# wjqkkky/TTS

Hardware: AMD Instinct MI355X
Metric: mel-frames/s (Tacotron2-DDC + MB-MelGAN end-to-end) (higher is better)
Workload: dtype f32; 1 GPU; C2: Tacotron2-DDC (r_init=7, r=2, sigmoid attn) + MB-MelGAN [8,4,2]x4, 32 LJ-length utterances per GPU; global_batch=32, r=2, parallelism=replicas x1

## Files before the change

### include/ttship.h

```cpp
#ifndef TTSHIP_H
#define TTSHIP_H

#include <stdint.h>

#ifdef __cplusplus
extern "C" {
#endif

typedef struct tts_ctx tts_ctx;

int tts_version(void);
const char* tts_last_error(void);

int tts_ctx_create(int device, tts_ctx** out);
int tts_ctx_destroy(tts_ctx* ctx);

int tts_taco_set_tensor(tts_ctx* ctx, const char* name, const float* h_data, const int64_t* shape, int ndim);
int tts_taco_finalize(tts_ctx* ctx, int num_chars, int r_init, int attn_norm);

int tts_taco_infer(tts_ctx* ctx, const int64_t* d_ids, const int32_t* h_lens, int B, int T_max, int r,
                   const int32_t* h_max_steps, int S_cap, float stop_threshold, float* d_dec, float* d_post,
                   float* d_align, float* d_stop, int32_t* h_steps, int32_t* h_status, void* stream);

int tts_taco_infer_spk(tts_ctx* ctx, const int64_t* d_ids, const int32_t* h_lens, int B, int T_max, int r,
// ... 85 lines not shown
                      int use_lstm_with_projection);
int tts_ge2e_infer(tts_ctx* ctx, const float* d_x, const int32_t* h_lens, int B, int T_max, float* d_out,
                   void* stream);

int tts_mel_to_linear(tts_ctx* ctx, const float* d_mel, const int32_t* h_lens, int B, int M_max, int n_mels,
                      int n_freq, const float* d_inv_basis, const float* d_scale, const float* d_offset,
                      float clip_lo, float clip_hi, int use_clip, float spec_gain, float power, float* d_S,
                      void* stream);

int tts_griffin_lim(tts_ctx* ctx, const float* d_S, const int32_t* h_lens, int B, int M_max, int n_fft,
                    int win_length, int hop_length, int iters, const float* d_phase0, float* d_wav, void* stream);

int tts_stft_mag(tts_ctx* ctx, const float* d_wav, const int32_t* h_nsamples, int B, int L_max, int n_fft,
                 int win_length, int hop_length, float preemphasis, int algo, float* d_mag, int M_max,
                 void* stream);

int tts_mag_to_feature(tts_ctx* ctx, const float* d_mag, const int32_t* h_lens, int B, int M_max, int n_freq,
                       int n_out, const float* d_basis, float spec_gain, const float* d_scale,
                       const float* d_offset, float clip_lo, float clip_hi, int use_clip, float* d_out,
                       void* stream);

int tts_spec_to_mag(tts_ctx* ctx, const float* d_spec, const int32_t* h_lens, int B, int M_max, int n_freq,
                    const float* d_scale, const float* d_offset, float clip_lo, float clip_hi, int use_clip,
                    float spec_gain, float power, float* d_S, void* stream);

int tts_deemphasis(tts_ctx* ctx, const float* d_in, const int32_t* h_nsamples, int B, int L_max, double a,
                   float* d_out, void* stream);

int tts_wav_finish(tts_ctx* ctx, const float* d_wav, const int32_t* h_nsamples, int B, int L_max,
                   int window_length, int hop_length, double threshold, int gap, int16_t* d_pcm, int32_t* d_ends,
                   int32_t* d_total, void* stream);

int tts_time_decoder_kernel(tts_ctx* ctx, int which, int iters, float* ms_out);

int tts_decoder_stats(tts_ctx* ctx, int* path, int* nlaunch, float* ms, int* steps);

int tts_set_gemm_mode(tts_ctx* ctx, int mode);
int tts_gemm_mode(tts_ctx* ctx, int* mode, int64_t* fallbacks);

int tts_taco_mbmelgan_infer(tts_ctx* ctx, const int64_t* d_ids, const int32_t* h_lens, int B, int T_max, int r,
                            const int32_t* h_max_steps, int S_cap, float thr, const int64_t* d_spk_ids,
                            const float* d_spk_emb, float* d_dec, float* d_post, float* d_align, float* d_stop,
                            int pad, float* d_wav, int32_t* h_steps, int32_t* h_status, void* stream);

int tts_taco_mbmelgan_submit(tts_ctx* ctx, const int64_t* d_ids, const int32_t* h_lens, int B, int T_max, int r,
                             const int32_t* h_max_steps, int S_cap, float thr, const int64_t* d_spk_ids,
                             const float* d_spk_emb, float* d_dec, float* d_post, float* d_align, float* d_stop,
                             int pad, float* d_wav, int32_t* h_steps, int32_t* h_status, int64_t* h_ticket,
                             void* stream);
int tts_taco_mbmelgan_finish(tts_ctx* ctx, int64_t ticket, void* stream);

int tts_test_stall_lstm(int recurrence);

#ifdef __cplusplus
}
#endif
#endif
```

### tts_amd/_lib.py

```python

import atexit
import collections
import ctypes
import os
import threading
from typing import Dict

import numpy as np

_HERE = os.path.dirname(os.path.abspath(__file__))
LIB_PATH = os.environ.get("TTSHIP_LIB", os.path.join(_HERE, "libttship.so"))

_lib = None
_lock = threading.Lock()

_c_int_p = ctypes.POINTER(ctypes.c_int32)
_c_i64_p = ctypes.POINTER(ctypes.c_int64)
_c_f_p = ctypes.POINTER(ctypes.c_float)
_c_i_p = ctypes.POINTER(ctypes.c_int)
_vp = ctypes.c_void_p

SIGNATURES = [
    ("tts_version", ctypes.c_int, []),
    ("tts_last_error", ctypes.c_char_p, []),
# ... 16 lines not shown
                                            _c_int_p, _vp]),
    ("tts_taco_forward_style", ctypes.c_int, [_vp, _vp, _c_int_p, ctypes.c_int, ctypes.c_int, ctypes.c_int, _vp,
                                              _c_int_p, ctypes.c_int, _vp, _vp, _vp, _vp, _vp, _vp, _vp, _vp]),
    ("tts_taco_mbmelgan_infer", ctypes.c_int, [_vp, _vp, _c_int_p, ctypes.c_int, ctypes.c_int, ctypes.c_int,
                                               _c_int_p, ctypes.c_int, ctypes.c_float, _vp, _vp, _vp, _vp, _vp,
                                               _vp, ctypes.c_int, _vp, _c_int_p, _c_int_p, _vp]),
    ("tts_taco_mbmelgan_submit", ctypes.c_int, [_vp, _vp, _c_int_p, ctypes.c_int, ctypes.c_int, ctypes.c_int,
                                                _c_int_p, ctypes.c_int, ctypes.c_float, _vp, _vp, _vp, _vp, _vp,
                                                _vp, ctypes.c_int, _vp, _c_int_p, _c_int_p, _c_i64_p, _vp]),
    ("tts_taco_mbmelgan_finish", ctypes.c_int, [_vp, ctypes.c_int64, _vp]),
    ("tts_taco_speaker_dim", ctypes.c_int, [_vp, _c_i_p, _c_i_p]),
    ("tts_taco_set_options", ctypes.c_int, [_vp, ctypes.c_int, ctypes.c_int, ctypes.c_int]),
    ("tts_taco_encoder", ctypes.c_int, [_vp, _vp, _c_int_p, ctypes.c_int, ctypes.c_int, _vp, _vp]),
    ("tts_taco_postnet", ctypes.c_int, [_vp, _vp, _c_int_p, ctypes.c_int, ctypes.c_int, _vp, _vp]),
    ("tts_taco_decoder_state", ctypes.c_int, [_vp, ctypes.c_int, ctypes.c_int, _vp, _vp, _vp, _vp, _vp, _vp, _vp, _vp]),
    ("tts_tacotron1_set_tensor", ctypes.c_int, [_vp, ctypes.c_char_p, _vp, _c_i64_p, ctypes.c_int]),
    ("tts_tacotron1_finalize", ctypes.c_int, [_vp, ctypes.c_int, ctypes.c_int, ctypes.c_int, ctypes.c_int,
                                              ctypes.c_int]),
    ("tts_tacotron1_infer", ctypes.c_int, [_vp, _vp, _c_int_p, ctypes.c_int, ctypes.c_int, ctypes.c_int, _c_int_p,
                                           ctypes.c_int, _vp, _vp, _vp, _vp, _c_int_p, _c_int_p, _vp]),
    ("tts_tacotron1_encoder", ctypes.c_int, [_vp, _vp, _c_int_p, ctypes.c_int, ctypes.c_int, _vp, _vp]),
    ("tts_tacotron1_postnet", ctypes.c_int, [_vp, _vp, _c_int_p, ctypes.c_int, ctypes.c_int, _vp, _vp]),
    ("tts_melgan_set_tensor", ctypes.c_int, [_vp, ctypes.c_char_p, _vp, _c_i64_p, ctypes.c_int]),
    ("tts_melgan_finalize", ctypes.c_int, [_vp, ctypes.c_int, ctypes.c_int, ctypes.c_int, _c_int_p, ctypes.c_int,
                                           ctypes.c_int, ctypes.c_int]),
    ("tts_melgan_infer", ctypes.c_int, [_vp, _vp, _c_int_p, ctypes.c_int, ctypes.c_int, ctypes.c_int, _vp, _vp]),
    ("tts_melgan_infer_strided", ctypes.c_int, [_vp, _vp, ctypes.c_int64, ctypes.c_int64, ctypes.c_int64, _c_int_p,
                                                ctypes.c_int, ctypes.c_int, ctypes.c_int, _vp, _vp]),
    ("tts_melgan_generator", ctypes.c_int, [_vp, _vp, _c_int_p, ctypes.c_int, ctypes.c_int, ctypes.c_int, _vp,
                                            _vp]),
    ("tts_pqmf_synthesis", ctypes.c_int, [_vp, _vp, ctypes.c_int, ctypes.c_int, ctypes.c_int, _vp, ctypes.c_int,
                                          _vp, _vp]),
    ("tts_ge2e_set_tensor", ctypes.c_int, [_vp, ctypes.c_char_p, _vp, _c_i64_p, ctypes.c_int]),
    ("tts_ge2e_finalize", ctypes.c_int, [_vp, ctypes.c_int, ctypes.c_int, ctypes.c_int, ctypes.c_int,
                                         ctypes.c_int]),
    ("tts_ge2e_infer", ctypes.c_int, [_vp, _vp, _c_int_p, ctypes.c_int, ctypes.c_int, _vp, _vp]),
    ("tts_pwgan_set_tensor", ctypes.c_int, [_vp, ctypes.c_char_p, _vp, _c_i64_p, ctypes.c_int]),
    ("tts_pwgan_finalize", ctypes.c_int, [_vp, ctypes.c_int, ctypes.c_int, _c_int_p, ctypes.c_int]),
    ("tts_pwgan_infer", ctypes.c_int, [_vp, _vp, _c_int_p, ctypes.c_int, ctypes.c_int, ctypes.c_int, _vp, _vp,
                                       _vp]),
    ("tts_glow_set_tensor", ctypes.c_int, [_vp, ctypes.c_char_p, _vp, _c_i64_p, ctypes.c_int]),
    ("tts_glow_finalize", ctypes.c_int, [_vp, ctypes.c_int, ctypes.c_int, ctypes.c_int, ctypes.c_int]),
    ("tts_glow_encode", ctypes.c_int, [_vp, _vp, _c_int_p, ctypes.c_int, ctypes.c_int, ctypes.c_float, _c_int_p,
                                       _vp]),
    ("tts_glow_encode_spk", ctypes.c_int, [_vp, _vp, _c_int_p, _c_int_p, ctypes.c_int, ctypes.c_int, ctypes.c_float,
                                           _c_int_p, _vp]),
    ("tts_glow_decode", ctypes.c_int, [_vp, _vp, ctypes.c_float, ctypes.c_int, _vp, _vp, _vp, _vp, _vp]),
    ("tts_glow_align", ctypes.c_int, [_vp, _vp, _c_int_p, ctypes.c_int, _vp, _vp, _vp, _vp, _vp, _vp, _vp, _vp]),
    ("tts_glow_mas", ctypes.c_int, [_vp, _vp, _c_int_p, _c_int_p, ctypes.c_int, ctypes.c_int, ctypes.c_int, _vp, _vp]),
    ("tts_time_decoder_kernel", ctypes.c_int, [_vp, ctypes.c_int, ctypes.c_int, _c_f_p]),
    ("tts_decoder_stats", ctypes.c_int, [_vp, _c_i_p, _c_i_p, _c_f_p, _c_i_p]),
    ("tts_set_gemm_mode", ctypes.c_int, [_vp, ctypes.c_int]),
    ("tts_test_stall_lstm", ctypes.c_int, [ctypes.c_int]),
    ("tts_gemm_mode", ctypes.c_int, [_vp, _c_i_p, _c_i64_p]),
    ("tts_mel_to_linear", ctypes.c_int, [_vp, _vp, _c_int_p, ctypes.c_int, ctypes.c_int, ctypes.c_int, ctypes.c_int,
                                         _vp, _vp, _vp, ctypes.c_float, ctypes.c_float, ctypes.c_int, ctypes.c_float,
                                         ctypes.c_float, _vp, _vp]),
    ("tts_griffin_lim", ctypes.c_int, [_vp, _vp, _c_int_p, ctypes.c_int, ctypes.c_int, ctypes.c_int, ctypes.c_int,
                                       ctypes.c_int, ctypes.c_int, _vp, _vp, _vp]),
    ("tts_stft_mag", ctypes.c_int, [_vp, _vp, _c_int_p, ctypes.c_int, ctypes.c_int, ctypes.c_int, ctypes.c_int,
                                    ctypes.c_int, ctypes.c_float, ctypes.c_int, _vp, ctypes.c_int, _vp]),
    ("tts_mag_to_feature", ctypes.c_int, [_vp, _vp, _c_int_p, ctypes.c_int, ctypes.c_int, ctypes.c_int, ctypes.c_int,
                                          _vp, ctypes.c_float, _vp, _vp, ctypes.c_float, ctypes.c_float, ctypes.c_int,
                                          _vp, _vp]),
    ("tts_spec_to_mag", ctypes.c_int, [_vp, _vp, _c_int_p, ctypes.c_int, ctypes.c_int, ctypes.c_int, _vp, _vp,
                                       ctypes.c_float, ctypes.c_float, ctypes.c_int, ctypes.c_float, ctypes.c_float,
                                       _vp, _vp]),
    ("tts_deemphasis", ctypes.c_int, [_vp, _vp, _c_int_p, ctypes.c_int, ctypes.c_int, ctypes.c_double, _vp, _vp]),
    ("tts_wav_finish", ctypes.c_int, [_vp, _vp, _c_int_p, ctypes.c_int, ctypes.c_int, ctypes.c_int, ctypes.c_int,
                                      ctypes.c_double, ctypes.c_int, _vp, _vp, _vp, _vp]),
]


def load_library():
    global _lib
    with _lock:
        if _lib is None:
            if not os.path.exists(LIB_PATH):
                raise RuntimeError(f"libttship.so not found at {LIB_PATH}; run __graft_entry__.build() "
                                   f"(make -C tts_amd/csrc)")
            lib = ctypes.CDLL(LIB_PATH)
            for name, res, args in SIGNATURES:
                fn = getattr(lib, name)
                fn.restype = res
                fn.argtypes = args
            _lib = lib
    return _lib


def _check(rc: int):
    if rc != 0:
        msg = load_library().tts_last_error()
        raise RuntimeError("ttship: " + (msg.decode() if msg else "unknown error"))


def _i32(a):
    arr = np.ascontiguousarray(np.asarray(a, dtype=np.int32))
    return arr, arr.ctypes.data_as(_c_int_p)


def _ptr(t):
    return ctypes.c_void_p(t.data_ptr())


def _opt_ptr(t):
    return None if t is None else _ptr(t)
# ... 246 lines not shown
        B, N, L = x.shape
        taps = G.shape[-1] - 1
        _check(self.lib.tts_pqmf_synthesis(self.h, _ptr(x), B, N, L, _ptr(G), taps, _ptr(y), _stream(x.device)))

    def mel_to_linear(self, mel, lens, inv_basis, scale, offset, clip, spec_gain, power, S):
        B, M, n_mels = mel.shape
        lens_a, lens_p = _i32(lens)
        lo, hi = (0.0, 0.0) if clip is None else clip
        _check(self.lib.tts_mel_to_linear(self.h, _ptr(mel), lens_p, B, M, n_mels, S.shape[-1], _ptr(inv_basis),
                                          _ptr(scale), _ptr(offset), float(lo), float(hi), int(clip is not None),
                                          float(spec_gain), float(power), _ptr(S), _stream(mel.device)))

    def griffin_lim(self, S, lens, n_fft, win_length, hop_length, iters, phase0, wav):
        B, M, _ = S.shape
        lens_a, lens_p = _i32(lens)
        _check(self.lib.tts_griffin_lim(self.h, _ptr(S), lens_p, B, M, int(n_fft), int(win_length), int(hop_length),
                                        int(iters), _ptr(phase0), _ptr(wav), _stream(S.device)))

    def stft_mag(self, wav, nsamples, n_fft, win_length, hop_length, preemphasis, mag, algo=0):
        B, L = wav.shape
        n_a, n_p = _i32(nsamples)
        _check(self.lib.tts_stft_mag(self.h, _ptr(wav), n_p, B, L, int(n_fft), int(win_length), int(hop_length),
                                     float(preemphasis), int(algo), _ptr(mag), mag.shape[1], _stream(wav.device)))

    def mag_to_feature(self, mag, lens, basis, spec_gain, scale, offset, clip, out):
        B, M, n_freq = mag.shape
        lens_a, lens_p = _i32(lens)
        lo, hi = (0.0, 0.0) if clip is None else clip
        _check(self.lib.tts_mag_to_feature(self.h, _ptr(mag), lens_p, B, M, n_freq, out.shape[-1],
                                           None if basis is None else _ptr(basis), float(spec_gain), _ptr(scale),
                                           _ptr(offset), float(lo), float(hi), int(clip is not None), _ptr(out),
                                           _stream(mag.device)))

    def spec_to_mag(self, spec, lens, scale, offset, clip, spec_gain, power, S):
        B, M, n_freq = spec.shape
        lens_a, lens_p = _i32(lens)
        lo, hi = (0.0, 0.0) if clip is None else clip
        _check(self.lib.tts_spec_to_mag(self.h, _ptr(spec), lens_p, B, M, n_freq, _ptr(scale), _ptr(offset),
                                        float(lo), float(hi), int(clip is not None), float(spec_gain), float(power),
                                        _ptr(S), _stream(spec.device)))

    def deemphasis(self, wav, nsamples, a, out):
        B, L = wav.shape
        n_a, n_p = _i32(nsamples)
        _check(self.lib.tts_deemphasis(self.h, _ptr(wav), n_p, B, L, float(a), _ptr(out), _stream(wav.device)))

    def wav_finish(self, wav, nsamples, window_length, hop_length, threshold, gap, pcm, ends, total):
        B, L = wav.shape
        n_a, n_p = _i32(nsamples)
        _check(self.lib.tts_wav_finish(self.h, _ptr(wav), n_p, B, L, int(window_length), int(hop_length),
                                       float(threshold), int(gap), _ptr(pcm), _ptr(ends), _ptr(total),
                                       _stream(wav.device)))

    def decoder_stats(self):
        path, n = ctypes.c_int(0), ctypes.c_int(0)
        ms = (ctypes.c_float * 4)()
        st = (ctypes.c_int * 4)()
        _check(self.lib.tts_decoder_stats(self.h, ctypes.byref(path), ctypes.byref(n), ms, st))
        return int(path.value), [(float(ms[i]), int(st[i])) for i in range(n.value)]

    def set_gemm_mode(self, mode: str):
        if mode not in ("x3", "f32"):
            raise ValueError("gemm mode must be 'x3' or 'f32'")
        with self.lock:
            _check(self.lib.tts_set_gemm_mode(self.h, 1 if mode == "x3" else 0))

    def gemm_mode(self):
        m, n = ctypes.c_int(0), ctypes.c_int64(0)
        _check(self.lib.tts_gemm_mode(self.h, ctypes.byref(m), ctypes.byref(n)))
        return ("x3" if m.value else "f32"), int(n.value)

    def time_decoder_kernel(self, which: int, iters: int) -> float:
        ms = ctypes.c_float(0.0)
        _check(self.lib.tts_time_decoder_kernel(self.h, which, iters, ctypes.byref(ms)))
        return float(ms.value)


_engines: Dict[int, Engine] = {}


def get_engine(device) -> Engine:
    import torch
    dev = torch.device(device)
    if dev.type != "cuda":
        raise RuntimeError("tts_amd runs on MI355X (ROCm 'cuda' devices) only; got device "
                           f"'{dev}'. There is no CPU fallback: move the model with .cuda().")
    idx = dev.index if dev.index is not None else torch.cuda.current_device()
    with _lock:
        eng = _engines.get(idx)
    if eng is None:
        eng = Engine(idx)
        with _lock:
            _engines[idx] = eng
    return eng


@atexit.register
def _close_engines():
    with _lock:
        engines = list(_engines.values())
        _engines.clear()
    for eng in engines:
        try:
            eng.close()
        except Exception:
            pass
# ... 1 lines not shown
```

### tts_amd/csrc/api_core.hip

```cpp
#include "host.h"
#include "split16.h"
#include "switches.h"

#include <cmath>
#include <cstring>
#include <memory>

static thread_local std::string g_err;
void tts_set_error(const std::string& m) { g_err = m; }

namespace ttsh {

__global__ void put_rows_kernel(int* dst, RowInts r, int n) {
  if ((int)threadIdx.x < n) dst[threadIdx.x] = r.v[threadIdx.x];
}

const int* put_rows(int* dst, const int32_t* h, int n, hipStream_t s) {
  for (int o = 0; o < n; o += BMAX) {
    const int m = std::min(BMAX, n - o);
    put_rows_kernel<<<1, BMAX, 0, s>>>(dst + o, row_ints(h + o, m), m);
    HIP_OK(hipGetLastError());
  }
  return dst;
}
// ... 274 lines not shown
    for (auto& e : c->ev_dec) HIP_OK(hipEventCreate(&e));
    HIP_OK(hipEventCreateWithFlags(&c->ev_status, hipEventDisableTiming));
    for (auto& t : c->vt) HIP_OK(hipEventCreateWithFlags(&t.ev, hipEventDisableTiming));
    HIP_OK(hipHostMalloc(reinterpret_cast<void**>(&c->pinned), PIN_N * 4, hipHostMallocDefault));
    std::memset(c->pinned, 0, PIN_N * 4);
    *out = c.release();
  });
}

int tts_ctx_destroy(tts_ctx* c) {
  return guarded([&] {
    if (!c) return;
    { std::lock_guard<std::recursive_mutex> lk(c->mu); }
    {
      DeviceGuard g(c->device);
      (void)hipStreamSynchronize(c->sv);
      (void)hipStreamSynchronize(c->s);
      for (auto& ge : c->tws.graphs)
        if (ge) {
          (void)hipGraphExecDestroy(ge);
          ge = nullptr;
        }
    }
    int dev = c->device;
    {
      DeviceGuard g(dev);
      hipStream_t s = c->s, sv = c->sv;
      std::vector<hipEvent_t> e = {c->ev_in, c->ev_out, c->ev_chunk[0], c->ev_chunk[1], c->ev_sv};
      for (auto ev : c->ev_dec) e.push_back(ev);
      e.push_back(c->ev_status);
      for (auto& t : c->vt) e.push_back(t.ev);
      int* pin = c->pinned;
      delete c;
      for (auto ev : e) (void)hipEventDestroy(ev);
      if (sv && sv != s) (void)hipStreamDestroy(sv);
      (void)hipStreamDestroy(s);
      (void)hipHostFree(pin);
    }
  });
}

int tts_set_gemm_mode(tts_ctx* c, int mode) {
  return guarded_ctx(c, [&] {
    TTS_CHECK(mode == 0 || mode == 1, "gemm mode must be 0 (fp32) or 1 (split-f16)");
    c->gemm_x3 = mode == 1;
  });
}

int tts_test_stall_lstm(int recurrence) {
  g_test_stall_lstm.store(recurrence < 0 ? -1 : recurrence);
  return 0;
}

int tts_gemm_mode(tts_ctx* c, int* mode, int64_t* fallbacks) {
  return guarded_ctx(c, [&] {
    TTS_CHECK(mode && fallbacks, "null argument");
    *mode = c->gemm_x3 ? 1 : 0;
    *fallbacks = c->x3_fallbacks;
  });
}

}
```

### tts_amd/csrc/conv_x3.hip

```cpp
#include "common.h"
#include "conv_epi.h"
#include "split16.h"
#include "switches.h"
#include "x3_tile.h"

#include <algorithm>
#include <mutex>
#include <map>

namespace {
constexpr int CX_XR = 80;
}

template <int MI, int NI, int WM, int WN, int KT, int RS, int SD>
__global__ __launch_bounds__(64 * WM * WN) void conv_x3_kernel(ConvArgs a, int nq, int nco, int nz) {
  constexpr int NTHR = 64 * WM * WN;
  constexpr int TC = 16 * MI * WM, TQ = 16 * NI * WN;
  constexpr int SPT = (4 * (TQ + CONV_MAX_SPAN) + NTHR - 1) / NTHR;
  static_assert(RS == KT || RS == 2 * KT, "weight ring: one or two chunks of taps");
  extern __shared__ __attribute__((aligned(16))) _Float16 shx[];

  const int ntile = nq * nco * nz;
  const int per = (ntile + 7) / 8;
  const int w = (int)(blockIdx.x % 8) * per + (int)(blockIdx.x / 8);
  if (w >= ntile) return;
  const int cot = w / (nq * nz);
  const int rem = w - cot * nq * nz;
  const int z = rem / nq;
  const int qt = rem - z * nq;

  const int ph = z % a.nphase;
  const int b = z / a.nphase;
  const int base = a.lens[b] + a.len_add;
  const int Lq = base * a.q_mul + (a.merged_u ? 1 : 0);
  const int q0 = qt * TQ;
  if (q0 >= Lq) return;
  const int co0 = cot * TC;
  const int Lin = base * a.in_mul;
  const int dil = a.dil;
  const int span = (KT - 1) * dil;
  const int ROWS = TQ + span;
  _Float16* X0 = shx;
  _Float16* X1 = shx + ROWS * CX_XR;

  const int tid = threadIdx.x;
  const int lane = tid & 63, wave = __builtin_amdgcn_readfirstlane(tid >> 6);
  const int wm = wave / WN, wn = wave % WN;
  const int nb = wn * 16 * NI + (lane & 15);
  const int kg = 8 * (lane >> 4);
  const int NCH = (a.Cin + 31) / 32;
  const int NKS = NCH * KT;
  const int mtiles = (a.Cout + 15) / 16;
  bool bad = false;

  const ConvSrc& S = a.src[0];
  const int i0 = q0 - a.pad_left[ph];
  const bool interior = (a.rep_pad == 0) && i0 >= 0 && i0 + ROWS <= Lin;
  const int rawL = a.lens[b];
  const int Lsrc = a.rep_pad ? rawL : Lin;
  const bool tmajor = S.sc == 1;
  const __amdgpu_buffer_rsrc_t xr = __builtin_amdgcn_make_buffer_rsrc(
      const_cast<float*>(S.ptr + (long)b * S.sb), 0,
      (int)min((long)0x7fffffff, ((long)(S.C - 1) * S.sc + (long)(Lsrc - 1) * S.st + 1) * 4), 0x00020000);
  int voff[SPT], sgv[SPT], srow[SPT];
  bool sval[SPT];
// ... 77 lines not shown
  stage_store(X0, st[0], 0);
  if constexpr (SD == 2) {
    if (NCH > 1) stage_load(st[1], 1);
    if (NCH > 2) stage_load(st[0], 2);
  }
  lds_barrier();
  for (int ch0 = 0; ch0 < NCH; ch0 += 2) {
#pragma unroll
    for (int p = 0; p < 2; ++p) {
      const int ch = ch0 + p;
      if (ch < NCH) {
        const _Float16* X = p ? X1 : X0;
        if constexpr (SD == 1) {
          if (ch + 1 < NCH) stage_load(st[0], ch + 1);
          __builtin_amdgcn_sched_barrier(0);
        }
#pragma unroll
        for (int kq = 0; kq < KT; ++kq) {
          constexpr bool TWO = RS == 2 * KT;
          const int slot = TWO ? p * KT + kq : kq;
          h8 bh[NI], bl[NI];
#pragma unroll
          for (int ni = 0; ni < NI; ++ni) {
            const _Float16* q = X + (nb + ni * 16 + kq * dil) * CX_XR + kg;
            bh[ni] = *reinterpret_cast<const h8*>(q);
            bl[ni] = *reinterpret_cast<const h8*>(q + 32);
          }
          __builtin_amdgcn_sched_barrier(0);
#pragma unroll
          for (int mi = 0; mi < MI; ++mi)
#pragma unroll
            for (int ni = 0; ni < NI; ++ni)
              mfma_x3(ring[slot][mi][0], ring[slot][mi][1], bh[ni], bl[ni], am[mi][ni], ac[mi][ni]);
          wload(ring[slot], ch * KT + kq + RS);
          __builtin_amdgcn_sched_barrier(0);
        }
        if constexpr (SD == 2) {
          if (ch + 1 < NCH) stage_store(p ? X0 : X1, st[p ^ 1], ch + 1);
          if (ch + 3 < NCH) stage_load(st[p ^ 1], ch + 3);
        } else {
          if (ch + 1 < NCH) stage_store(p ? X0 : X1, st[0], ch + 1);
        }
        lds_barrier();
      }
    }
  }
  f32x4 acc[MI][NI];
#pragma unroll
  for (int mi = 0; mi < MI; ++mi)
#pragma unroll
    for (int ni = 0; ni < NI; ++ni)
#pragma unroll
      for (int j = 0; j < 4; ++j) acc[mi][ni][j] = x3_value(am[mi][ni][j], ac[mi][ni][j]);
  const bool vec = a.merged_u && a.ot == 1 && (a.oc & 3) == 0 && (a.ob & 3) == 0 &&
                   (reinterpret_cast<uintptr_t>(a.out) & 15) == 0 && a.Cout % 16 == 0;
  if (vec && a.merged_u % 4 == 0) {
    const int u = a.merged_u, L = Lin;
    float* ob = a.out + (long)b * a.ob;
#pragma unroll
    for (int mi = 0; mi < MI; ++mi) {
      const int m0 = co0 + wm * 16 * MI + mi * 16 + 4 * (lane >> 4);
      if (m0 >= a.Cout) continue;
      const int co = m0 / u, phs0 = m0 - co * u;
      const int hi0 = 2 * phs0 >= u, hi1 = 2 * (phs0 + 2) >= u;
      const f32x4 bias{a.bias[m0], a.bias[m0 + 1], a.bias[m0 + 2], a.bias[m0 + 3]};
      float* orow = ob + (long)co * a.oc;
#pragma unroll
      for (int ni = 0; ni < NI; ++ni) {
        const int q = q0 + nb + ni * 16;
        const f32x4 v = acc[mi][ni] + bias;
        if (u % 8 == 0) {
          if (q - hi0 >= 0 && q - hi0 < L) *reinterpret_cast<f32x4*>(orow + (long)(q - hi0) * u + phs0) = v;
        } else {
          typedef float f2 __attribute__((ext_vector_type(2)));
          if (q - hi0 >= 0 && q - hi0 < L) *reinterpret_cast<f2*>(orow + (long)(q - hi0) * u + phs0) = f2{v[0], v[1]};
          if (q - hi1 >= 0 && q - hi1 < L) *reinterpret_cast<f2*>(orow + (long)(q - hi1) * u + phs0 + 2) = f2{v[2], v[3]};
        }
      }
    }
  } else if (vec && a.merged_u == 2) {
    typedef float f2 __attribute__((ext_vector_type(2)));
    const int L = Lin;
    float* ob = a.out + (long)b * a.ob;
    const int r = lane & 15;
#pragma unroll
    for (int mi = 0; mi < MI; ++mi) {
      const int m0 = co0 + wm * 16 * MI + mi * 16 + 4 * (lane >> 4);
      if (m0 >= a.Cout) continue;
#pragma unroll
      for (int c = 0; c < 2; ++c) {
        const int co = m0 / 2 + c;
        const float b0 = a.bias[m0 + 2 * c], b1 = a.bias[m0 + 2 * c + 1];
        float* orow = ob + (long)co * a.oc;
#pragma unroll
        for (int ni = 0; ni < NI; ++ni) {
          const float v0 = acc[mi][ni][2 * c] + b0;
          const float v1 = acc[mi][ni][2 * c + 1] + b1;
          const float down = __shfl_down(v1, 1, 16);
          const float wrap = ni + 1 < NI ? __shfl(acc[mi][ni + 1 < NI ? ni + 1 : ni][2 * c + 1] + b1, lane & ~15) : 0.f;
          const int q = q0 + nb + ni * 16;
          const bool last = r == 15 && ni == NI - 1;
          if (q >= 0 && q < L) {
            if (last) orow[2 * q] = v0;
            else *reinterpret_cast<f2*>(orow + 2 * q) = f2{v0, r < 15 ? down : wrap};
          }
          if (r == 0 && ni == 0 && q - 1 >= 0 && q - 1 < L) orow[2 * q - 1] = v1;
        }
      }
    }
  } else if (a.merged_u) {
    const int u = a.merged_u, L = Lin;
    float* ob = a.out + (long)b * a.ob;
#pragma unroll
    for (int mi = 0; mi < MI; ++mi)
#pragma unroll
      for (int j = 0; j < 4; ++j) {
        const int m = co0 + wm * 16 * MI + mi * 16 + 4 * (lane >> 4) + j;
        if (m >= a.Cout) continue;
        const int co = m / u, phs = m - co * u;
        const int hi = 2 * phs >= u;
        const float bias = a.bias[m];
#pragma unroll
        for (int ni = 0; ni < NI; ++ni) {
          const int qq = q0 + nb + ni * 16 - hi;
#ifdef CX_PROBE_NOSTORE
          if (qq >= 0 && qq < L && acc[mi][ni][j] + bias == 12345.f) ob[(long)co * a.oc + (long)(qq * u + phs) * a.ot] = 0.f;
#else
          if (qq >= 0 && qq < L) ob[(long)co * a.oc + (long)(qq * u + phs) * a.ot] = acc[mi][ni][j] + bias;
#endif
        }
      }
  } else {
    conv_epilogue<MI, NI, WN>(a, acc, b, ph, q0, co0, wm, wn, lane);
  }
  if (bad) __hip_atomic_fetch_or(a.oflow, 1u, __ATOMIC_RELAXED, __HIP_MEMORY_SCOPE_AGENT);
}

enum { CX_T128 = 0, CX_T192, CX_T96, CX_T64, CX_T80, CX_T48, CX_NONE };

static int cx_tile(int Cout) {
  if (Cout % 128 == 0) return CX_T128;
  if (Cout == 192) return CX_T192;
  if (Cout == 96) return CX_T96;
  if (Cout == 80) return CX_T80;
  if (Cout == 48) return CX_T48;
  if (Cout % 64 == 0) return CX_T64;
  if (Cout % 80 == 0) return CX_T80;
  return CX_NONE;
}

bool conv_x3_supported(int Cin, int Cout, int K, int dil) {
  return Cin % 8 == 0 && Cin >= 8 && cx_tile(Cout) != CX_NONE && (K == 1 || K == 2 || K == 3 || K == 5 || K == 7) &&
         (K - 1) * dil <= CONV_MAX_SPAN;
}

template <int MI, int NI, int WM, int WN, int KT, int RS, int SD>
static void cx_launch(const ConvArgs& a, hipStream_t s) {
  constexpr int TC = 16 * MI * WM, TQ = 16 * NI * WN;
  ensure_dyn_lds((const void*)conv_x3_kernel<MI, NI, WM, WN, KT, RS, SD>, 160 * 1024);
  const int nq = (a.max_q + TQ - 1) / TQ, nco = (a.Cout + TC - 1) / TC, nz = a.B * a.nphase;
  const long ntile = (long)nq * nco * nz;
  TTS_CHECK(ntile < (1L << 30), "conv_x3: grid too large");
  const int per = (int)((ntile + 7) / 8);
  const size_t lds = (size_t)2 * (TQ + (KT - 1) * a.dil) * CX_XR * 2;
  conv_x3_kernel<MI, NI, WM, WN, KT, RS, SD><<<dim3(8 * per), 64 * WM * WN, lds, s>>>(a, nq, nco, nz);
}

template <int MI, int NI, int WM, int WN, int KT, int RS, int SD>
static long cx_cost_k(const ConvArgs& a) {
  constexpr int TC = 16 * MI * WM, TQ = 16 * NI * WN;
  const void* f = (const void*)conv_x3_kernel<MI, NI, WM, WN, KT, RS, SD>;
  const size_t lds = (size_t)2 * (TQ + (KT - 1) * a.dil) * CX_XR * 2;
  static std::mutex mu;
  static std::map<size_t, long> slots_by_lds;
  long slots;
  ensure_dyn_lds(f, 160 * 1024);
  const int cus = device_cu_count();
  {
    std::lock_guard<std::mutex> lk(mu);
    auto it = slots_by_lds.find(lds);
    if (it == slots_by_lds.end()) {
      int nb = 0;
      HIP_OK(hipOccupancyMaxActiveBlocksPerMultiprocessor(&nb, f, 64 * WM * WN, lds));
      it = slots_by_lds.emplace(lds, std::max(1L, (long)nb * cus)).first;
    }
    slots = it->second;
  }
  const long tiles = (long)((a.max_q + TQ - 1) / TQ) * ((a.Cout + TC - 1) / TC) * a.B * a.nphase;
  return (tiles + slots - 1) / slots * TQ;
}
template <int MI, int NI, int WM, int WN, int SD12>
static long cx_cost(const ConvArgs& a) {
  switch (a.K) {
    case 1: return cx_cost_k<MI, NI, WM, WN, 1, 2, SD12>(a);
    case 2: return cx_cost_k<MI, NI, WM, WN, 2, 2 * SD12, SD12>(a);
    case 3: return cx_cost_k<MI, NI, WM, WN, 3, 3, 1>(a);
    case 5: return cx_cost_k<MI, NI, WM, WN, 5, 5, 2>(a);
    case 7: return cx_cost_k<MI, NI, WM, WN, 7, 7, 1>(a);
    default: return 0;
  }
}

template <int MI, int NI, int WM, int WN, int SD12>
static void cx_taps(const ConvArgs& a, hipStream_t s) {
  switch (a.K) {
    case 1: cx_launch<MI, NI, WM, WN, 1, 2, SD12>(a, s); break;
    case 2: cx_launch<MI, NI, WM, WN, 2, 2 * SD12, SD12>(a, s); break;
    case 3: cx_launch<MI, NI, WM, WN, 3, 3, 1>(a, s); break;
    case 5: cx_launch<MI, NI, WM, WN, 5, 5, 2>(a, s); break;
    case 7: cx_launch<MI, NI, WM, WN, 7, 7, 1>(a, s); break;
    default: TTS_CHECK(false, "conv_x3: unsupported tap count");
  }
}

void launch_conv_x3(const ConvArgs& a, hipStream_t s) {
  TTS_CHECK(conv_x3_supported(a.Cin, a.Cout, a.K, a.dil), "conv_x3: unsupported shape");
  TTS_CHECK(a.W16 && a.oflow, "conv_x3: split weights / overflow flag missing");
// ... 52 lines not shown
```

### tts_amd/csrc/switches.h

```cpp
#pragma once
#include <cstdlib>
#include <string>

namespace sw {

inline bool on_unless_zero(const char* name, bool dflt) {
  const char* e = std::getenv(name);
  return e ? std::atoi(e) != 0 : dflt;
}
inline bool on_unless_one(const char* name) {
  const char* e = std::getenv(name);
  return !e || std::atoi(e) != 1;
}
inline bool present(const char* name) { return std::getenv(name) != nullptr; }
inline int number(const char* name, int dflt) {
  const char* e = std::getenv(name);
  return e ? std::atoi(e) : dflt;
}
inline std::string text(const char* name) {
  const char* e = std::getenv(name);
  return e ? e : "";
}

inline bool gemm_f32() { static const bool v = text("TTS_GEMM") == "f32"; return v; }
inline bool voc_stream() { static const bool v = on_unless_zero("TTS_VOC_STREAM", true); return v; }

inline double barrier_timeout_ms() {
  static const double v = [] {
    const char* e = std::getenv("TTS_BARRIER_TIMEOUT_MS");
    const double ms = e ? std::atof(e) : 2000.0;
    return ms < 1.0 ? 1.0 : (ms > 40000.0 ? 40000.0 : ms);
  }();
  return v;
}
inline bool coop_launch() { static const bool v = on_unless_zero("TTS_COOP_LAUNCH", false); return v; }
inline bool bar_calibrate() { static const bool v = on_unless_zero("TTS_BAR_CALIBRATE", true); return v; }
inline bool diag_xcc() { static const bool v = present("TTS_DIAG_XCC"); return v; }

inline bool encoder_steps() { static const bool v = text("TTS_ENCODER") == "steps"; return v; }
inline bool lstm_row_groups() { static const bool v = on_unless_one("TTS_LSTM_RG"); return v; }
inline bool decoder_graph() { static const bool v = text("TTS_DECODER") == "graph"; return v; }
inline bool decoder_f32() { static const bool v = present("TTS_DECODER_F32"); return v; }
inline bool align_in_p4() { static const bool v = present("TTS_ALIGN_IN_P4"); return v; }
inline const char* ptrace_file() {
  static const bool set = present("TTS_PTRACE");
  static const std::string v = text("TTS_PTRACE");
  return set ? v.c_str() : nullptr;
}
inline int ptrace_t0() { static const int v = number("TTS_PTRACE_T0", 100); return v; }
inline int ptrace_launch() { static const int v = number("TTS_PTRACE_LAUNCH", 0); return v; }

inline bool stack_fuse() { static const bool v = on_unless_zero("TTS_STACK_FUSE", true); return v; }
inline bool stack_fuse96() { static const bool v = on_unless_zero("TTS_STACK_FUSE96", false); return v; }
inline bool ct_fuse() { static const bool v = on_unless_zero("TTS_CT_FUSE", true); return v; }
inline int cx_ni128() { static const int v = number("TTS_CX_NI128", 0); return v; }

inline bool ge2e_pipe() { static const bool v = text("TTS_GE2E_PIPE") != "0"; return v; }

inline int pwgan_staging() {
  static const int v = [] {
    const std::string e = text("TTS_PWGAN_STAGING");
    return e == "regs" ? 0 : e == "ring4" ? 2 : 1;
  }();
  return v;
}
inline int pwgan_tile() { static const int v = number("TTS_PWGAN_TILE", 0); return v; }

}
```

### tts_amd/csrc/x3_tile.h

```cpp
#pragma once
#include "common.h"
#include "split16.h"

__device__ __forceinline__ __amdgpu_buffer_rsrc_t x3_rsrc(const void* p) {
  return __builtin_amdgcn_make_buffer_rsrc(const_cast<void*>(p), 0, 0x7fffffff, 0x00020000);
}

__device__ __forceinline__ void x3_load_a(h8 (&r)[2], __amdgpu_buffer_rsrc_t w, int wlo, int blk) {
  r[0] = __builtin_bit_cast(h8, __builtin_amdgcn_raw_buffer_load_b128(w, wlo, blk, 0));
  r[1] = __builtin_bit_cast(h8, __builtin_amdgcn_raw_buffer_load_b128(w, wlo + 16, blk, 0));
}

struct X3Tile {
  int b, q0, L;
};
template <int TQ>
__device__ __forceinline__ void x3_tile_scan(int* tcum, int* tlen, int lane, int L) {
  const int n = (L + TQ - 1) / TQ;
  int v = n;
#pragma unroll
  for (int o = 1; o < 64; o <<= 1) {
    const int y = __shfl_up(v, o, 64);
    if (lane >= o) v += y;
  }
  tcum[lane] = v - n;
  tlen[lane] = L;
  if (lane == 63) tcum[64] = v;
}
template <int TQ>
__device__ __forceinline__ X3Tile x3_tile_of(const int* tcum, const int* tlen, int B, int lane, int i) {
  const bool hit = lane < B && tcum[lane] <= i && i < tcum[lane + 1];
  const unsigned long long m = __ballot(hit);
  const int b = __builtin_amdgcn_readfirstlane(m ? __ffsll((long long)m) - 1 : 0);
  X3Tile r;
  r.b = b;
  r.q0 = __builtin_amdgcn_readfirstlane((i - tcum[b]) * TQ);
  r.L = __builtin_amdgcn_readfirstlane(tlen[b]);
  return r;
}

inline long x3_tile_count(const int* h_lens, int B, int len_add, int mul, int TQ, const char* who) {
  long ntiles = 0;
  for (int b = 0; b < B; ++b) ntiles += ((long)(h_lens[b] + len_add) * mul + TQ - 1) / TQ;
  TTS_CHECK(ntiles < (1L << 30), std::string(who) + ": too many tiles");
  return ntiles;
}
```

Baseline: 1.321 million mel-frames/s.

## Add persistent conv_x3 kernel that prefetches next tile during epilogue

```diff
diff --git a/include/ttship.h b/include/ttship.h
--- a/include/ttship.h
+++ b/include/ttship.h
@@ -161,6 +161,10 @@
 
 int tts_test_stall_lstm(int recurrence);
 
+int tts_test_conv1d(tts_ctx* ctx, const float* d_x, const int32_t* h_lens, int B, int T_max, int bound, int Cin,
+                    int Cout, int K, int up, const float* h_w, const float* h_bias, float* d_y, int* h_flag,
+                    void* stream);
+
 #ifdef __cplusplus
 }
 #endif
diff --git a/tts_amd/_lib.py b/tts_amd/_lib.py
--- a/tts_amd/_lib.py
+++ b/tts_amd/_lib.py
@@ -92,6 +92,8 @@
     ("tts_decoder_stats", ctypes.c_int, [_vp, _c_i_p, _c_i_p, _c_f_p, _c_i_p]),
     ("tts_set_gemm_mode", ctypes.c_int, [_vp, ctypes.c_int]),
     ("tts_test_stall_lstm", ctypes.c_int, [ctypes.c_int]),
+    ("tts_test_conv1d", ctypes.c_int, [_vp, _vp, _c_int_p, ctypes.c_int, ctypes.c_int, ctypes.c_int, ctypes.c_int,
+                                       ctypes.c_int, ctypes.c_int, ctypes.c_int, _c_f_p, _c_f_p, _vp, _c_i_p, _vp]),
     ("tts_gemm_mode", ctypes.c_int, [_vp, _c_i_p, _c_i64_p]),
     ("tts_mel_to_linear", ctypes.c_int, [_vp, _vp, _c_int_p, ctypes.c_int, ctypes.c_int, ctypes.c_int, ctypes.c_int,
                                          _vp, _vp, _vp, ctypes.c_float, ctypes.c_float, ctypes.c_int, ctypes.c_float,
@@ -444,6 +446,18 @@
                                        float(threshold), int(gap), _ptr(pcm), _ptr(ends), _ptr(total),
                                        _stream(wav.device)))
 
+    def test_conv1d(self, x, lens, bound, weight, bias, up, y):
+        B, Cin, T = x.shape
+        w = np.ascontiguousarray(weight, dtype=np.float32)
+        b = np.ascontiguousarray(bias, dtype=np.float32)
+        Cout, K = (w.shape[1], w.shape[2]) if up else (w.shape[0], w.shape[2])
+        lens_a, lens_p = _i32(lens)
+        flag = ctypes.c_int(0)
+        _check(self.lib.tts_test_conv1d(self.h, _ptr(x), lens_p, B, T, int(bound), Cin, Cout, K, int(up),
+                                        w.ctypes.data_as(_c_f_p), b.ctypes.data_as(_c_f_p), _ptr(y),
+                                        ctypes.byref(flag), _stream(x.device)))
+        return int(flag.value)
+
     def decoder_stats(self):
         path, n = ctypes.c_int(0), ctypes.c_int(0)
         ms = (ctypes.c_float * 4)()
diff --git a/tts_amd/csrc/api_core.hip b/tts_amd/csrc/api_core.hip
--- a/tts_amd/csrc/api_core.hip
+++ b/tts_amd/csrc/api_core.hip
@@ -350,6 +350,55 @@
   return 0;
 }
 
+int tts_test_conv1d(tts_ctx* c, const float* d_x, const int32_t* h_lens, int B, int T_max, int bound, int Cin,
+                    int Cout, int K, int up, const float* h_w, const float* h_bias, float* d_y, int* h_flag,
+                    void* stream) {
+  return guarded_ctx(c, [&] {
+    TTS_CHECK(d_x && h_lens && h_w && h_bias && d_y && h_flag, "null argument");
+    TTS_CHECK(B >= 1 && B <= BMAX && T_max >= 1 && Cin >= 16 && Cin % 16 == 0 && Cout >= 1, "bad sizes");
+    TTS_CHECK(up == 0 ? (K == 1 || K == 3 || K == 5 || K == 7) : (up % 2 == 0 && up <= 8 && K == 2 * up),
+              "Conv1d with k = 1, 3, 5, 7, or ConvTranspose1d with k = 2 up, up even and <= 8");
+    check_rows(h_lens, B, 1, std::min(T_max, bound), "test_conv1d: lens out of range");
+    DeviceGuard g(c->device);
+    enter(c, stream);
+    hipStream_t s = c->s;
+    ConvLayer L;
+    DevBuf lens;
+    const int* dl = put_rows(lens, h_lens, B, s);
+    unsigned* flag = x3_flag(c);
+    if (flag) HIP_OK(hipMemsetAsync(flag, 0, 4, s));
+    const std::vector<float> bias(h_bias, h_bias + Cout);
+    if (up == 0) {
+      const int pl[8] = {(K - 1) / 2};
+      pack_conv(L, std::vector<float>(h_w, h_w + (size_t)Cout * Cin * K), bias, Cin, Cout, K, 1, 1, pl);
+      run_conv(L, conv_call(c, dl, B, bound).in(d_x, bct(Cin, T_max), Cin).to(d_y, bct(Cout, T_max)), s);
+    } else {
+      TTS_CHECK(flag && conv_x3_supported(Cin, up * Cout, 2, 1), "test_conv1d: ConvTranspose1d shape not covered");
+      const int p = up / 2;
+      std::vector<float> Wm((size_t)up * Cout * Cin * 2), bm((size_t)up * Cout);
+      for (int ph = 0; ph < up; ++ph) {
+        const int dmin = (ph + p) / up - 1;
+        for (int co = 0; co < Cout; ++co)
+          for (int ci = 0; ci < Cin; ++ci)
+            for (int jj = 0; jj < 2; ++jj)
+              Wm[(((size_t)ph * Cout + co) * Cin + ci) * 2 + jj] =
+                  h_w[((size_t)ci * Cout + co) * (2 * up) + ph + p - (dmin + jj) * up];
+      }
+      for (size_t r = 0; r < bm.size(); ++r) bm[r] = bias[r / up];
+      pack_conv_x3_only(L, merge_convT_phases(Wm, up, Cin, Cout), bm, Cin, up * Cout, 2);
+      ConvCall t = conv_call(c, dl, B, bound + 1);
+      t.in(d_x, bct(Cin, T_max), Cin).to(d_y, bct(Cout, (long)T_max * up));
+      t.merged_u = up;
+      run_conv(L, t, s);
+    }
+    int raised = 0;
+    if (flag) HIP_OK(hipMemcpyAsync(&raised, flag, 4, hipMemcpyDeviceToHost, s));
+    HIP_OK(hipStreamSynchronize(s));
+    *h_flag = raised;
+    leave(c, stream);
+  });
+}
+
 int tts_gemm_mode(tts_ctx* c, int* mode, int64_t* fallbacks) {
   return guarded_ctx(c, [&] {
     TTS_CHECK(mode && fallbacks, "null argument");
diff --git a/tts_amd/csrc/conv_x3.hip b/tts_amd/csrc/conv_x3.hip
--- a/tts_amd/csrc/conv_x3.hip
+++ b/tts_amd/csrc/conv_x3.hip
@@ -7,10 +7,15 @@
 #include <algorithm>
 #include <mutex>
 #include <map>
+#include <tuple>
 
 namespace {
 constexpr int CX_XR = 80;
 }
+
+template <int MI, int NI, int WN>
+__device__ __forceinline__ void cx_epilogue(const ConvArgs& a, f32x4 (&acc)[MI][NI], int b, int ph, int q0, int co0,
+                                            int Lin, int wm, int wn, int lane);
 
 template <int MI, int NI, int WM, int WN, int KT, int RS, int SD>
 __global__ __launch_bounds__(64 * WM * WN) void conv_x3_kernel(ConvArgs a, int nq, int nco, int nz) {
@@ -194,6 +199,14 @@
     for (int ni = 0; ni < NI; ++ni)
 #pragma unroll
       for (int j = 0; j < 4; ++j) acc[mi][ni][j] = x3_value(am[mi][ni][j], ac[mi][ni][j]);
+  cx_epilogue<MI, NI, WN>(a, acc, b, ph, q0, co0, Lin, wm, wn, lane);
+  if (bad) __hip_atomic_fetch_or(a.oflow, 1u, __ATOMIC_RELAXED, __HIP_MEMORY_SCOPE_AGENT);
+}
+
+template <int MI, int NI, int WN>
+__device__ __forceinline__ void cx_epilogue(const ConvArgs& a, f32x4 (&acc)[MI][NI], int b, int ph, int q0, int co0,
+                                            int Lin, int wm, int wn, int lane) {
+  const int nb = wn * 16 * NI + (lane & 15);
   const bool vec = a.merged_u && a.ot == 1 && (a.oc & 3) == 0 && (a.ob & 3) == 0 &&
                    (reinterpret_cast<uintptr_t>(a.out) & 15) == 0 && a.Cout % 16 == 0;
   if (vec && a.merged_u % 4 == 0) {
@@ -275,6 +288,261 @@
   } else {
     conv_epilogue<MI, NI, WN>(a, acc, b, ph, q0, co0, wm, wn, lane);
   }
+}
+
+struct CxTile {
+  int b, ph, q0, co0, Lin;
+};
+template <class T>
+__device__ __forceinline__ const T* cx_uniform(const T* p) {
+  const unsigned long long v = reinterpret_cast<unsigned long long>(p);
+  const unsigned lo = __builtin_amdgcn_readfirstlane((unsigned)v);
+  const unsigned hi = __builtin_amdgcn_readfirstlane((unsigned)(v >> 32));
+  return reinterpret_cast<const T*>(((unsigned long long)hi << 32) | lo);
+}
+template <int MI, int NI, int WM, int WN, int KT, int RS, int SD>
+__global__ __launch_bounds__(64 * WM * WN) void conv_x3p_kernel(ConvArgs a, int nco) {
+  constexpr int NTHR = 64 * WM * WN;
+  constexpr int TC = 16 * MI * WM, TQ = 16 * NI * WN;
+  constexpr int SPT = (4 * (TQ + CONV_MAX_SPAN) + NTHR - 1) / NTHR;
+  static_assert(RS == KT || RS == 2 * KT, "weight ring: one or two chunks of taps");
+  extern __shared__ __attribute__((aligned(16))) _Float16 shx[];
+  __shared__ int tcum[65], tlen[64];
+
+  const int tid = threadIdx.x;
+  const int lane = tid & 63, wave = __builtin_amdgcn_readfirstlane(tid >> 6);
+  const int wm = wave / WN, wn = wave % WN;
+  const int nb = wn * 16 * NI + (lane & 15);
+  const int kg = 8 * (lane >> 4);
+  const int NCH = (a.Cin + 31) / 32;
+  const int NKS = NCH * KT;
+  const int mtiles = (a.Cout + 15) / 16;
+  const int dil = a.dil;
+  const int span = (KT - 1) * dil;
+  const int ROWS = TQ + span;
+  _Float16* X0 = shx;
+  _Float16* X1 = shx + ROWS * CX_XR;
+  bool bad = false;
+
+  if (wave == 0) {
+    int L = 0;
+    if (lane < a.B) L = max(0, min((a.lens[lane] + a.len_add) * a.q_mul + (a.merged_u ? 1 : 0), a.max_q));
+    x3_tile_scan<TQ>(tcum, tlen, lane, L);
+  }
+  lds_barrier();
+  const int T = __builtin_amdgcn_readfirstlane(tcum[64]);
+  const int N = nco * a.nphase * T;
+  const int G = (int)gridDim.x, nx = min(G, 8), xcd = (int)(blockIdx.x % 8), S = (G - xcd + 7) / 8;
+  const X3Walk walk = x3_walk(N, nx, xcd);
+  int u = (int)(blockIdx.x / 8);
+  if (u >= walk.n) return;
+  auto tile_of = [&](int uu) {
+    const int w = walk.lo + uu, per = a.nphase * T;
+    const int cot = w / per, i = w - cot * per, ph = i / T;
+    const X3Tile xt = x3_tile_of<TQ>(tcum, tlen, a.B, lane, i - ph * T);
+    CxTile t;
+    t.b = xt.b, t.ph = ph, t.q0 = xt.q0, t.co0 = cot * TC;
+    t.Lin = (a.lens[xt.b] + a.len_add) * a.in_mul;
+    return t;
+  };
+
+  const ConvSrc& S0 = a.src[0];
+  const bool tmajor = S0.sc == 1;
+  const int act = S0.act;
+  int sgv[SPT], srow[SPT], voff[SPT];
+  bool sval[SPT];
+#pragma unroll
+  for (int j = 0; j < SPT; ++j) {
+    const int e = tid + NTHR * j;
+    sgv[j] = e / ROWS;
+    srow[j] = e - sgv[j] * ROWS;
+  }
+  const float* xbase = S0.ptr;
+  int xbytes = 0;
+  auto stage_setup = [&](const CxTile& t) {
+    const int i0 = t.q0 - a.pad_left[t.ph];
+    const bool interior = (a.rep_pad == 0) && i0 >= 0 && i0 + ROWS <= t.Lin;
+    const int Lsrc = a.rep_pad ? a.lens[t.b] : t.Lin;
+    xbase = cx_uniform(S0.ptr + (long)t.b * S0.sb);
+    xbytes = __builtin_amdgcn_readfirstlane(
+        (int)min((long)0x7fffffff, ((long)(S0.C - 1) * S0.sc + (long)(Lsrc - 1) * S0.st + 1) * 4));
+#pragma unroll
+    for (int j = 0; j < SPT; ++j) {
+      int i = i0 + srow[j];
+      bool valid = true;
+      if (!interior) {
+        i = map_pad_index(i, t.Lin, a.pad_mode, valid);
+        if (a.rep_pad) i -= a.rep_pad;
+      }
+      i = i < 0 ? 0 : (i >= Lsrc ? Lsrc - 1 : i);
+      sval[j] = valid && sgv[j] < 4;
+      voff[j] = (min(sgv[j], 3) * 8 * S0.sc + i * S0.st) * 4;
+    }
+  };
+  float st[SD][SPT][8];
+  auto stage_load = [&](float (&sr)[SPT][8], int ch) {
+    const __amdgpu_buffer_rsrc_t xr =
+        __builtin_amdgcn_make_buffer_rsrc(const_cast<float*>(xbase), 0, xbytes, 0x00020000);
+    const int cb = 32 * ch * S0.sc * 4;
+#pragma unroll
+    for (int j = 0; j < SPT; ++j) {
+      if (tmajor) {
+        const f32x4 p = __builtin_bit_cast(f32x4, __builtin_amdgcn_raw_buffer_load_b128(xr, voff[j], cb, 0));
+        const f32x4 v = __builtin_bit_cast(f32x4, __builtin_amdgcn_raw_buffer_load_b128(xr, voff[j] + 16, cb, 0));
+#pragma unroll
+        for (int c = 0; c < 4; ++c) sr[j][c] = p[c], sr[j][4 + c] = v[c];
+      } else {
+#pragma unroll
+        for (int c = 0; c < 8; ++c)
+          sr[j][c] = __uint_as_float(__builtin_amdgcn_raw_buffer_load_b32(xr, voff[j], cb + c * S0.sc * 4, 0));
+      }
+    }
+  };
+  auto stage_store = [&](_Float16* X, const float (&sr)[SPT][8], int ch) {
+#pragma unroll
+    for (int j = 0; j < SPT; ++j) {
+      if (sgv[j] < 4) {
+        const bool keep = sval[j] && 32 * ch + 8 * sgv[j] < a.Cin;
+        float mx = 0.f, v[8];
+#pragma unroll
+        for (int c = 0; c < 8; ++c) {
+          v[c] = keep ? sr[j][c] : 0.f;
+          mx = fmaxf(mx, __builtin_fabsf(v[c]));
+          if (act) v[c] = lrelu02(v[c]);
+        }
+        bad |= !(mx < F16_RANGE);
+        h8 hi8, lo8;
+        split8(v, hi8, lo8);
+        *reinterpret_cast<h8*>(X + srow[j] * CX_XR + 8 * sgv[j]) = hi8;
+        *reinterpret_cast<h8*>(X + srow[j] * CX_XR + 32 + 8 * sgv[j]) = lo8;
+      }
+    }
+  };
+
+#ifdef CX_PROBE_NOPREFETCH
+  const bool wrap = false;
+#else
+  const bool wrap = NKS % RS == 0;
+#endif
+  const char* wcur = nullptr;
+  const char* wnxt = nullptr;
+  int mcur = 0, mnxt = 0;
+  const int wlo = lane * 32;
+  h8 ring[RS][MI][2];
+  auto wload = [&](h8 (&r)[MI][2], int seq) {
+    const bool over = wrap && seq >= NKS;
+    const __amdgpu_buffer_rsrc_t wr = x3_rsrc(cx_uniform(over ? wnxt : wcur));
+    const int m0 = __builtin_amdgcn_readfirstlane(over ? mnxt : mcur);
+    const int ks = over ? seq - NKS : min(seq, NKS - 1);
+#pragma unroll
+    for (int mi = 0; mi < MI; ++mi) {
+      const int mt = min(m0 + mi, mtiles - 1);
+      x3_load_a(r[mi], wr, wlo, (mt * NKS + ks) * 2048);
+    }
+  };
+  auto wbase = [&](const CxTile& t) { return reinterpret_cast<const char*>(a.W16) + (long)t.ph * a.w16_phase_stride; };
+
+  f32x4 am[MI][NI], ac[MI][NI];
+  auto kloop = [&]() {
+    for (int ch0 = 0; ch0 < NCH; ch0 += 2) {
+#pragma unroll
+      for (int p = 0; p < 2; ++p) {
+        const int ch = ch0 + p;
+        if (ch < NCH) {
+          const _Float16* X = p ? X1 : X0;
+          if constexpr (SD == 1) {
+            if (ch + 1 < NCH) stage_load(st[0], ch + 1);
+            __builtin_amdgcn_sched_barrier(0);
+          }
+#pragma unroll
+          for (int kq = 0; kq < KT; ++kq) {
+            constexpr bool TWO = RS == 2 * KT;
+            const int slot = TWO ? p * KT + kq : kq;
+            h8 bh[NI], bl[NI];
+#pragma unroll
+            for (int ni = 0; ni < NI; ++ni) {
+              const _Float16* q = X + (nb + ni * 16 + kq * dil) * CX_XR + kg;
+              bh[ni] = *reinterpret_cast<const h8*>(q);
+              bl[ni] = *reinterpret_cast<const h8*>(q + 32);
+            }
+            __builtin_amdgcn_sched_barrier(0);
+#pragma unroll
+            for (int mi = 0; mi < MI; ++mi)
+#pragma unroll
+              for (int ni = 0; ni < NI; ++ni)
+                mfma_x3(ring[slot][mi][0], ring[slot][mi][1], bh[ni], bl[ni], am[mi][ni], ac[mi][ni]);
+            wload(ring[slot], ch * KT + kq + RS);
+            __builtin_amdgcn_sched_barrier(0);
+          }
+          if constexpr (SD == 2) {
+            if (ch + 1 < NCH) stage_store(p ? X0 : X1, st[p ^ 1], ch + 1);
+            if (ch + 3 < NCH) stage_load(st[p ^ 1], ch + 3);
+          } else {
+            if (ch + 1 < NCH) stage_store(p ? X0 : X1, st[0], ch + 1);
+          }
+          lds_barrier();
+        }
+      }
+    }
+  };
+  auto stage_first = [&]() {
+    stage_store(X0, st[0], 0);
+    if constexpr (SD == 2) {
+      if (NCH > 1) stage_load(st[1], 1);
+      if (NCH > 2) stage_load(st[0], 2);
+    }
+    lds_barrier();
+  };
+
+  CxTile cur = tile_of(u);
+  wcur = wnxt = wbase(cur);
+  mcur = mnxt = cur.co0 / 16 + wm * MI;
+  stage_setup(cur);
+  stage_load(st[0], 0);
+#pragma unroll
+  for (int r = 0; r < RS; ++r) wload(ring[r], r);
+  stage_first();
+  for (;;) {
+    const int un = u + S;
+    const bool more = un < walk.n;
+    const CxTile nxt = more ? tile_of(un) : cur;
+    wnxt = wbase(nxt);
+    mnxt = nxt.co0 / 16 + wm * MI;
+#pragma unroll
+    for (int mi = 0; mi < MI; ++mi)
+#pragma unroll
+      for (int ni = 0; ni < NI; ++ni) am[mi][ni] = ac[mi][ni] = f32x4{0.f, 0.f, 0.f, 0.f};
+    kloop();
+    auto next_first = [&]() {
+      stage_setup(nxt);
+      stage_load(st[0], 0);
+      wcur = wnxt, mcur = mnxt;
+      if (!wrap) {
+#pragma unroll
+        for (int r = 0; r < RS; ++r) wload(ring[r], r);
+      }
+    };
+#ifndef CX_PROBE_NOPREFETCH
+    next_first();
+#endif
+    f32x4 acc[MI][NI];
+#pragma unroll
+    for (int mi = 0; mi < MI; ++mi)
+#pragma unroll
+      for (int ni = 0; ni < NI; ++ni)
+#pragma unroll
+        for (int j = 0; j < 4; ++j) acc[mi][ni][j] = x3_value(am[mi][ni][j], ac[mi][ni][j]);
+    int le = lane;
+    asm volatile("" : "+v"(le));
+    cx_epilogue<MI, NI, WN>(a, acc, cur.b, cur.ph, cur.q0, cur.co0, cur.Lin, wm, wn, le);
+    if (!more) break;
+#ifdef CX_PROBE_NOPREFETCH
+    next_first();
+#endif
+    cur = nxt;
+    u = un;
+    stage_first();
+  }
   if (bad) __hip_atomic_fetch_or(a.oflow, 1u, __ATOMIC_RELAXED, __HIP_MEMORY_SCOPE_AGENT);
 }
 
@@ -296,6 +564,26 @@
          (K - 1) * dil <= CONV_MAX_SPAN;
 }
 
+static int cx_resident(const void* f, int threads, size_t lds) {
+  static std::mutex mu;
+  static std::map<std::tuple<const void*, size_t, int>, int> fits;
+  int dev = 0;
+  HIP_OK(hipGetDevice(&dev));
+  std::lock_guard<std::mutex> lk(mu);
+  auto it = fits.find({f, lds, dev});
+  if (it == fits.end()) {
+    int nb = 0;
+    HIP_OK(hipOccupancyMaxActiveBlocksPerMultiprocessor(&nb, f, threads, lds));
+    it = fits.emplace(std::make_tuple(f, lds, dev), nb).first;
+  }
+  return it->second;
+}
+
+constexpr int CXP_DYN_LDS = 159 * 1024;
+
+template <int MI, int NI, int WM, int WN, int KT>
+constexpr bool cx_persistent_tile = MI == 2 && NI == 3 && WM == 4 && WN == 1 && KT == 5;
+
 template <int MI, int NI, int WM, int WN, int KT, int RS, int SD>
 static void cx_launch(const ConvArgs& a, hipStream_t s) {
   constexpr int TC = 16 * MI * WM, TQ = 16 * NI * WN;
@@ -305,6 +593,20 @@
   TTS_CHECK(ntile < (1L << 30), "conv_x3: grid too large");
   const int per = (int)((ntile + 7) / 8);
   const size_t lds = (size_t)2 * (TQ + (KT - 1) * a.dil) * CX_XR * 2;
+  if constexpr (cx_persistent_tile<MI, NI, WM, WN, KT>) {
+    if (sw::cx_persist() && a.B <= 64 && lds <= (size_t)CXP_DYN_LDS) {
+      const void* fp = (const void*)conv_x3p_kernel<MI, NI, WM, WN, KT, RS, SD>;
+      ensure_dyn_lds(fp, CXP_DYN_LDS);
+      const int occ_p = cx_resident(fp, 64 * WM * WN, lds);
+      const int occ_t = cx_resident((const void*)conv_x3_kernel<MI, NI, WM, WN, KT, RS, SD>, 64 * WM * WN, lds);
+      if (occ_p >= 1 && occ_p >= occ_t) {
+        long grid = std::min<long>(ntile, (long)occ_p * device_cu_count());
+        if (sw::cx_grid() > 0) grid = std::min<long>(grid, sw::cx_grid());
+        conv_x3p_kernel<MI, NI, WM, WN, KT, RS, SD><<<dim3((unsigned)grid), 64 * WM * WN, lds, s>>>(a, nco);
+        return;
+      }
+    }
+  }
   conv_x3_kernel<MI, NI, WM, WN, KT, RS, SD><<<dim3(8 * per), 64 * WM * WN, lds, s>>>(a, nq, nco, nz);
 }
 
diff --git a/tts_amd/csrc/switches.h b/tts_amd/csrc/switches.h
--- a/tts_amd/csrc/switches.h
+++ b/tts_amd/csrc/switches.h
@@ -54,6 +54,8 @@
 inline bool stack_fuse96() { static const bool v = on_unless_zero("TTS_STACK_FUSE96", false); return v; }
 inline bool ct_fuse() { static const bool v = on_unless_zero("TTS_CT_FUSE", true); return v; }
 inline int cx_ni128() { static const int v = number("TTS_CX_NI128", 0); return v; }
+inline bool cx_persist() { static const bool v = on_unless_zero("TTS_CX_PERSIST", true); return v; }
+inline int cx_grid() { static const int v = number("TTS_CX_GRID", 0); return v; }
 
 inline bool ge2e_pipe() { static const bool v = text("TTS_GE2E_PIPE") != "0"; return v; }
 
diff --git a/tts_amd/csrc/x3_tile.h b/tts_amd/csrc/x3_tile.h
--- a/tts_amd/csrc/x3_tile.h
+++ b/tts_amd/csrc/x3_tile.h
@@ -39,6 +39,16 @@
   return r;
 }
 
+struct X3Walk {
+  int lo, n;
+};
+__host__ __device__ inline X3Walk x3_walk(int N, int nx, int x) {
+  X3Walk w;
+  w.lo = (int)((long)N * x / nx);
+  w.n = (int)((long)N * (x + 1) / nx) - w.lo;
+  return w;
+}
+
 inline long x3_tile_count(const int* h_lens, int B, int len_add, int mul, int TQ, const char* who) {
   long ntiles = 0;
   for (int b = 0; b < B; ++b) ntiles += ((long)(h_lens[b] + len_add) * mul + TQ - 1) / TQ;
```

After: 1.323 million mel-frames/s, median of 2. No clear change (+0.1%).
